# CRIMAC-WP4-Machine-learning/CRIMAC-classifiers-unet

Hardware: AMD Instinct MI355X
Metric: echogram patches/sec (4ch 256x256), training step (fwd+weighted CE+bwd+SGD) (higher is better)
Workload: dtype bf16; 1 GPU; BASELINE configs[1]: U-Net (depth 5, 64 filters) train step, batch 32 x 4x256x256 per GPU; global_batch=32, precision=bf16, start_filts=64, parallelism=dp1, ranks=1, launcher=single process

## Files before the change

### crimac_classifiers_unet_amd/csrc/wgrad.hip

```cpp
#include "common.h"

CRIMAC_DIAG_DECLARE(crimac_diag_clock_wgrad)

namespace {

struct WgradParams {
  const void* f; long f_ld; int CF;
  const void* s; long s_ld; int CS;
  int B, Hf, Wf;
  float* dw;
  int tiles_y, tiles_x;
  long ntiles;
  int tiles_per_block;
  int nsplits;
  long partial_stride;
  int f_es = 2, s_es = 2;
};

__device__ __forceinline__ int swz_tr(int row) { return ((row >> 1) & 1) << 6; }

__device__ __forceinline__ bf16x4 lds_tr16(const unsigned char* p) {
  return __builtin_amdgcn_ds_read_tr16_b64_v4bf16((LDS_PTR(bf16x4))(p));
}

// ... 936 lines not shown
        s_pixel(row, y0, x0, y, x);
        const bool ok = y >= 0 && y < Hs && x >= 0 && x < Ws && (cs0 + u * 8) < p.CS;
        const TA* src = sp + ((b * Hs + y) * (long)Ws + x) * p.s_ld + cs0 + u * 8;
        stage_unit(src, ok, sS, S_BYTES, row * 128 + ((u * 16) ^ swz_tr(row)));
      }
      __syncthreads();
      contract(sF, sS);
    }
  }

  const int col = cs0 + ws * 32 + (lane & 31);
#ifdef CRIMAC_EXP_NOATOMIC
  if (col < 0) {
#else
  if (col < p.CS) {
#endif
    float* dwp = p.dw + (p.partial_stride > 0 ? (long)split * p.partial_stride : 0);
#pragma unroll
    for (int t = 0; t < NTAPS; ++t) {
#pragma unroll
      for (int r = 0; r < 16; ++r) {
        const int row = cf0 + wf * 32 + (r & 3) + 8 * (r >> 2) + 4 * (lane >> 5);
        if (row < p.CF) {
          float* dst = dwp + ((long)t * p.CF + row) * p.CS + col;
          if (p.partial_stride > 0) *dst = acc[t][r];
          else atomicAdd(dst, acc[t][r]);
        }
      }
    }
  }
}

constexpr int kGroupMaxLayers = CRIMAC_WGRAD_GROUP_MAX_LAYERS;
using GroupLayer = crimac_wgrad_group_layer;
struct GroupParams {
  GroupLayer layer[kGroupMaxLayers];
  int B;
  const int* items;
  int cap;
  int count[8];
  unsigned* counter;
  int f_es, s_es;
  int max_items;
};

__device__ __forceinline__ void group_barrier_lds() {
  asm volatile("s_waitcnt lgkmcnt(0)" ::: "memory");
  __builtin_amdgcn_s_barrier();
  asm volatile("" ::: "memory");
}

__device__ __forceinline__ unsigned lds_word(const unsigned* p) {
  return *(volatile LDS_PTR(unsigned))(LDS_PTR(unsigned))(p);
}

template <typename TA>
__global__ __launch_bounds__(512) __attribute__((amdgpu_waves_per_eu(2, 2)))
void wgrad_group_kernel(GroupParams gp) {
  constexpr int MODE = 0, TR = 8, NTAPS = 9;
  constexpr int F_ROWS = TR * 16;
  constexpr int S_ROWS = (TR + 2) * 18;
  constexpr int S_ROWS_PAD = (S_ROWS + 7) / 8 * 8;
  constexpr int F_BYTES = F_ROWS * 128;
  constexpr int S_BYTES = S_ROWS_PAD * 128;
  constexpr int BUF_BYTES = F_BYTES + S_BYTES;
  constexpr int NF = F_ROWS / 8 / 4;
  constexpr int NS = (S_ROWS_PAD / 8 + 3) / 4;
  constexpr unsigned OOB = 0x80000000u;
  extern __shared__ __attribute__((aligned(16))) unsigned char smem[];
  const int tid = threadIdx.x, lane = tid & 63;
  const int team = __builtin_amdgcn_readfirstlane(tid >> 8);
  const int wave = __builtin_amdgcn_readfirstlane((tid >> 6) & 3);
  const int ws = wave & 1, tg = wave >> 1;
  const int g = lane >> 4, li = lane & 15;
  const int q = li >> 2, pp = li & 3;
  const int sub = lane >> 3, c = lane & 7;
  const int xcd = blockIdx.x & 7;
  unsigned* tq = reinterpret_cast<unsigned*>(smem + 4 * BUF_BYTES);
  const int n_items = gp.count[xcd];
  auto fetch_item = [&](int par) {
    const unsigned k = __hip_atomic_fetch_add(gp.counter + xcd, 1u, __ATOMIC_RELAXED, __HIP_MEMORY_SCOPE_AGENT);
    unsigned a = 0, b = 0;
    if (k < (unsigned)n_items) {
      const int* it = gp.items + 2 * ((long)xcd * gp.cap + k);
      a = (unsigned)it[0];
      b = (unsigned)it[1];
    }
    tq[8 + 4 * par] = k;
    tq[9 + 4 * par] = a;
    tq[10 + 4 * par] = b;
  };
  if (tid == 256) fetch_item(0);
  __syncthreads();
  int ipar = 0;

  auto run = [&](auto tgc) {
    constexpr int TG = decltype(tgc)::value;
    using G = WgTaps<MODE, TG>;
    f32x4 acc2[G::N][4][2];
    const int RF = (g >> 1) * 16 + 4 * (g & 1) + q;
    const int RSl = (g >> 1) * G::RS + 4 * (g & 1) + q;
    const unsigned lds0 = (unsigned)(unsigned long)((LDS_PTR(unsigned char))(smem)) + team * 2 * BUF_BYTES;
    const int tt = tid & 255;
    unsigned* tcnt = tq + team;
    for (int taken = 0;; ++taken) {
      const int k = __builtin_amdgcn_readfirstlane((int)lds_word(tq + 8 + 4 * ipar));
      if (k >= n_items) break;
      const int li_ = __builtin_amdgcn_readfirstlane((int)lds_word(tq + 9 + 4 * ipar));
      const int qs = __builtin_amdgcn_readfirstlane((int)lds_word(tq + 10 + 4 * ipar));
      const GroupLayer& p = gp.layer[li_];
      const int qt = qs >> 16, split = qs & 0xFFFF;
      const int cs_tiles = (p.CS + 63) / 64;
      const int cf0 = (qt / cs_tiles) * 64, cs0 = (qt % cs_tiles) * 64;
      const TA* fp = reinterpret_cast<const TA*>(p.f);
      const TA* sp = reinterpret_cast<const TA*>(p.s);
      const int Hs = p.Hf, Ws = p.Wf;
#pragma unroll
      for (int t = 0; t < G::N; ++t)
#pragma unroll
        for (int fh = 0; fh < 4; ++fh)
#pragma unroll
          for (int sh = 0; sh < 2; ++sh)
#pragma unroll
            for (int r = 0; r < 4; ++r) acc2[t][fh][sh][r] = 0.f;
      unsigned f_rel[NF], s_rel[NS];
      auto f_geo = [&](int i, int& ry, int& rx) {
        const int row = 8 * (wave + 4 * i) + sub;
        ry = row >> 4;
        rx = row & 15;
      };
      auto s_geo = [&](int i, int& ry, int& rx) {
        const int row = 8 * (wave + 4 * i) + sub;
        ry = (row * 3641) >> 16;
        rx = row - ry * 18;
      };
#pragma unroll
      for (int i = 0; i < NF; ++i) {
        const int row = 8 * (wave + 4 * i) + sub;
        const int u = c ^ (swz16(row) >> 4);
        int ry, rx;
        f_geo(i, ry, rx);
        f_rel[i] = (cf0 + u * 8) < p.CF ? (unsigned)(((ry * (long)p.Wf + rx) * p.f_ld + cf0 + u * 8) * gp.f_es) : OOB;
      }
#pragma unroll
      for (int i = 0; i < NS; ++i) {
        const int kk = wave + 4 * i;
        const int row = 8 * kk + sub;
        const int u = c ^ (swz16(row) >> 4);
// ... 416 lines not shown
  hipStream_t st = (hipStream_t)stream;
  const bool two = teams_of(prec, mode) == 2;
  if (prec == CRIMAC_PREC_BF16) {
    if (mode == 0 && CS <= 16)
      return two ? launch<bf16_t, 1, 0, true, 2>(p, target_blocks, st) : launch<bf16_t, 1, 0, true>(p, target_blocks, st);
    if (mode == 0) return two ? launch<bf16_t, 1, 0, false, 2>(p, target_blocks, st) : launch<bf16_t, 1, 0>(p, target_blocks, st);
    return launch<bf16_t, 1, 1>(p, target_blocks, st);
  }
  if (prec == CRIMAC_PREC_FP16) {
    if (mode == 0 && CS <= 16)
      return two ? launch<half_t, 1, 0, true, 2>(p, target_blocks, st) : launch<half_t, 1, 0, true>(p, target_blocks, st);
    if (mode == 0) return two ? launch<half_t, 1, 0, false, 2>(p, target_blocks, st) : launch<half_t, 1, 0>(p, target_blocks, st);
    return launch<half_t, 1, 1>(p, target_blocks, st);
  }
  if (prec == CRIMAC_PREC_F32X3)
    return mode == 0 ? launch<float, 2, 0>(p, target_blocks, st) : launch<float, 2, 1>(p, target_blocks, st);
  if (prec == CRIMAC_PREC_H3P) {
    if (pp_ok(prec, mode, CF, CS, f_ld, s_ld, Wf)) return launch_pp(p, target_blocks, st);
    if (up_pp_ok(prec, mode, CF, CS, f_ld, s_ld, Wf, p.partial_stride)) return launch_up_pp(p, target_blocks, st);
    return mode == 0 ? launch<hp_t, 2, 0>(p, target_blocks, st) : launch<hp_t, 2, 1>(p, target_blocks, st);
  }
  return mode == 0 ? launch<float, 3, 0>(p, target_blocks, st) : launch<float, 3, 1>(p, target_blocks, st);
}

}

static int group_check(int prec, const crimac_wgrad_group_layer* L, int n, int B) {
  CRIMAC_REQUIRE(prec == CRIMAC_PREC_BF16 || prec == CRIMAC_PREC_FP16 || prec == CRIMAC_PREC_H3P || prec == CRIMAC_PREC_H3F_BWD,
                 "wgrad_group: 16-bit storage precisions, plane pairs and H3F_BWD only (prec=%d)", prec);
  const bool hp = prec == CRIMAC_PREC_H3P;
  const bool mix = prec == CRIMAC_PREC_H3F_BWD;
  CRIMAC_REQUIRE(L && n >= 1 && n <= CRIMAC_WGRAD_GROUP_MAX_LAYERS && B > 0, "wgrad_group: 1..%d layers", CRIMAC_WGRAD_GROUP_MAX_LAYERS);
  for (int i = 0; i < n; ++i) {
    CRIMAC_REQUIRE(L[i].CF > 0 && L[i].CF % 8 == 0 && L[i].CS >= 64 && L[i].CS % 8 == 0, "wgrad_group: layer %d: CF=%d CS=%d "
                   "(CS >= 64: the first layer keeps its own launch)", i, L[i].CF, L[i].CS);
    CRIMAC_REQUIRE(L[i].f_ld >= L[i].CF && L[i].s_ld >= L[i].CS && L[i].f_ld % 8 == 0 && L[i].s_ld % 8 == 0 && L[i].Hf > 0 && L[i].Wf > 0,
                   "wgrad_group: layer %d: bad strides / sizes", i);
    CRIMAC_REQUIRE((10L * L[i].Wf + 18) * (L[i].f_ld > L[i].s_ld ? L[i].f_ld : L[i].s_ld) * ((hp || mix) ? 4 : 2) < (1L << 31),
                   "wgrad_group: layer %d: a tile's DMA offsets exceed 32 bits", i);
    CRIMAC_REQUIRE(!hp || (L[i].CF % 64 == 0 && L[i].CS % 64 == 0), "wgrad_group: layer %d: plane pairs need whole 64-channel "
                   "tiles (CF=%d CS=%d)", i, L[i].CF, L[i].CS);
  }
  return CRIMAC_OK;
}

extern "C" int crimac_wgrad_group_layer_size(void) { return (int)sizeof(crimac_wgrad_group_layer); }

extern "C" int crimac_wgrad_group_plan(int prec, crimac_wgrad_group_layer* layers, int n_layers, int B, int items_per_layer,
                                       int* items, int cap, int* counts) {
  if (int rc = group_check(prec, layers, n_layers, B)) return rc;
  CRIMAC_REQUIRE(counts, "wgrad_group_plan: counts is NULL");
  static const int env_items = getenv("CRIMAC_WGRAD_GROUP_ITEMS") ? atoi(getenv("CRIMAC_WGRAD_GROUP_ITEMS")) : 0;
  const int target = items_per_layer > 0 ? items_per_layer : (env_items > 0 ? env_items : 128);
  int order[CRIMAC_WGRAD_GROUP_MAX_LAYERS];
  for (int i = 0; i < n_layers; ++i) {
    crimac_wgrad_group_layer& l = layers[i];
    l.tiles_y = cdiv(l.Hf, 8);
    l.tiles_x = cdiv(l.Wf, 16);
    l.ntiles = (long)B * l.tiles_y * l.tiles_x;
    const int ch_tiles = cdiv(l.CF, 64) * cdiv(l.CS, 64);
    long splits = target / ch_tiles;
    const long pix = (long)B * l.Hf * l.Wf;
    long max_splits = pix / 4096 > 1 ? pix / 4096 : 1;
    while (max_splits * ch_tiles < target / 2 && max_splits * 2 <= pix / 1024) max_splits *= 2;
    if (splits > max_splits) splits = max_splits;
    if (splits < 1) splits = 1;
    if (splits > l.ntiles) splits = l.ntiles;
    if (splits >= 8) splits = splits / 8 * 8;
    l.tiles_per_block = cdiv(l.ntiles, splits);
    l.nsplits = cdiv(l.ntiles, l.tiles_per_block);
    CRIMAC_REQUIRE(ch_tiles < 65536 && l.nsplits < 65536, "wgrad_group_plan: layer %d does not fit the item encoding", i);
    order[i] = i;
  }
  for (int a = 1; a < n_layers; ++a)
    for (int b = a; b > 0 && layers[order[b]].tiles_per_block > layers[order[b - 1]].tiles_per_block; --b) {
      const int t = order[b]; order[b] = order[b - 1]; order[b - 1] = t;
    }
  int n[8] = {0, 0, 0, 0, 0, 0, 0, 0};
  long rr = 0;
  for (int oi = 0; oi < n_layers; ++oi) {
    const int li = order[oi];
    const crimac_wgrad_group_layer& l = layers[li];
    const int ch_tiles = cdiv(l.CF, 64) * cdiv(l.CS, 64);
    auto put = [&](int x, int qt, int split) {
      if (items && n[x] < cap) {
        items[2 * ((long)x * cap + n[x])] = li;
        items[2 * ((long)x * cap + n[x]) + 1] = qt * 65536 + split;
      }
      ++n[x];
    };
    if (l.nsplits % 8 == 0) {
      for (int x = 0; x < 8; ++x)
        for (int sp = x; sp < l.nsplits; sp += 8)
          for (int qt = 0; qt < ch_tiles; ++qt) put(x, qt, sp);
    } else {
      for (int sp = 0; sp < l.nsplits; ++sp)
        for (int qt = 0; qt < ch_tiles; ++qt) put((int)(rr++ % 8), qt, sp);
    }
  }
  int need = 0;
  for (int x = 0; x < 8; ++x) { counts[x] = n[x]; if (n[x] > need) need = n[x]; }
  if (items) CRIMAC_REQUIRE(need <= cap, "wgrad_group_plan: %d items per queue, room for %d", need, cap);
  return need;
}

extern "C" int crimac_wgrad_group(int prec, const crimac_wgrad_group_layer* layers, int n_layers, int B, const int* items,
                                  int cap, const int* counts, unsigned int* counters, void* stream) {
  if (int rc = group_check(prec, layers, n_layers, B)) return rc;
  CRIMAC_REQUIRE(items && counts && counters && cap > 0, "wgrad_group: bad queue arguments");
  GroupParams gp;
  for (int i = 0; i < n_layers; ++i) {
    gp.layer[i] = layers[i];
    CRIMAC_REQUIRE(layers[i].f && layers[i].s && layers[i].dw, "wgrad_group: layer %d: NULL tensor", i);
    CRIMAC_REQUIRE(layers[i].tiles_per_block > 0 && layers[i].nsplits > 0 && layers[i].ntiles == (long)B * layers[i].tiles_y * layers[i].tiles_x &&
                       layers[i].tiles_y == cdiv(layers[i].Hf, 8) && layers[i].tiles_x == cdiv(layers[i].Wf, 16),
                   "wgrad_group: layer %d was not planned for this geometry (crimac_wgrad_group_plan)", i);
  }
  gp.B = B; gp.items = items; gp.cap = cap; gp.counter = counters;
  gp.f_es = 2; gp.s_es = prec == CRIMAC_PREC_H3F_BWD ? 4 : 2;
  long total = 0;
  for (int x = 0; x < 8; ++x) {
    CRIMAC_REQUIRE(counts[x] >= 0 && counts[x] <= cap, "wgrad_group: queue %d holds %d items, capacity %d", x, counts[x], cap);
    gp.count[x] = counts[x];
    total += counts[x];
  }
  if (total == 0) return CRIMAC_OK;
  constexpr size_t lds = 4 * (size_t)((8 * 16 + ((8 + 2) * 18 + 7) / 8 * 8) * 128) + 64;
  hipStream_t st = (hipStream_t)stream;
  int ncu = crimac_cu_count();
  ncu = ncu / 8 * 8;
  if (ncu < 8) ncu = 8;
  static const int wg_items = getenv("CRIMAC_WGRAD_GROUP_WGITEMS") ? atoi(getenv("CRIMAC_WGRAD_GROUP_WGITEMS")) : 1;
  gp.max_items = wg_items;
  if (wg_items > 0) {
    int per_xcd = 0;
    for (int x = 0; x < 8; ++x) { const int n = cdiv(counts[x], wg_items); if (n > per_xcd) per_xcd = n; }
    ncu = 8 * per_xcd;
  }
  if (prec == CRIMAC_PREC_H3P) {
    static unsigned long long attr_devs = 0;
    if (crimac_first_use_on_device(&attr_devs))
      (void)hipFuncSetAttribute(reinterpret_cast<const void*>(&wgrad_pp_group_kernel), hipFuncAttributeMaxDynamicSharedMemorySize, 160 * 1024);
    hipLaunchKernelGGL(wgrad_pp_group_kernel, dim3(ncu), dim3(512), 2 * (size_t)PP_BUF + 64, st, gp);
  } else if (prec == CRIMAC_PREC_BF16) {
    static unsigned long long attr_devs = 0;
    if (crimac_first_use_on_device(&attr_devs))
      (void)hipFuncSetAttribute(reinterpret_cast<const void*>(&wgrad_group_kernel<bf16_t>), hipFuncAttributeMaxDynamicSharedMemorySize, 160 * 1024);
    hipLaunchKernelGGL(wgrad_group_kernel<bf16_t>, dim3(ncu), dim3(512), lds, st, gp);
  } else {
    static unsigned long long attr_devs = 0;
    if (crimac_first_use_on_device(&attr_devs))
      (void)hipFuncSetAttribute(reinterpret_cast<const void*>(&wgrad_group_kernel<half_t>), hipFuncAttributeMaxDynamicSharedMemorySize, 160 * 1024);
    hipLaunchKernelGGL(wgrad_group_kernel<half_t>, dim3(ncu), dim3(512), lds, st, gp);
  }
  CRIMAC_LAUNCH_CHECK();
  return CRIMAC_OK;
}

extern "C" int crimac_wgrad(int prec, int mode, const void* f, long f_ld, int CF, const void* s,
                            long s_ld, int CS, int B, int Hf, int Wf, float* dw, int target_blocks,
                            void* stream) {
  return wgrad_run(prec, mode, f, f_ld, CF, s, s_ld, CS, B, Hf, Wf, dw, 0, target_blocks, stream);
}

extern "C" int crimac_wgrad_splits(int prec, int mode, int CF, int CS, int B, int Hf, int Wf, int target_blocks) {
  if (prec < CRIMAC_PREC_BF16 || prec > CRIMAC_PREC_MAX || !(mode == 0 || mode == 1) || CF <= 0 || CS <= 0 || B <= 0 ||
      Hf <= 0 || Wf <= 0)
    return CRIMAC_ERR_INVALID;
  WgradParams p;
  p.CF = CF; p.CS = CS; p.B = B; p.Hf = Hf; p.Wf = Wf;
  plan_splits(p, mode, target_blocks, pp_ok(prec, mode, CF, CS, CF, CS, Wf) ? 2 : teams_of(prec, mode));
  return p.nsplits;
}

extern "C" int crimac_wgrad_partials(int prec, int mode, const void* f, long f_ld, int CF, const void* s,
                                     long s_ld, int CS, int B, int Hf, int Wf, float* partials, long slab_stride,
                                     int target_blocks, void* stream) {
  CRIMAC_REQUIRE(slab_stride > 0, "wgrad_partials: slab_stride must be positive");
  return wgrad_run(prec, mode, f, f_ld, CF, s, s_ld, CS, B, Hf, Wf, partials, slab_stride, target_blocks, stream);
}
```

### crimac_classifiers_unet_amd/engine.py

```python
from __future__ import annotations

import ctypes as C
import os

import torch

from . import hip
from .hip import Act, call, ptr


def _on_device(fn):
    import functools

    @functools.wraps(fn)
    def wrapped(self, *a, **kw):
        if getattr(self, "device", None) is None:
            self.bind()
        dev = self.device
        if dev is None or dev.type != "cuda":
            return fn(self, *a, **kw)
        with torch.cuda.device(dev):
            return fn(self, *a, **kw)
    return wrapped

# ... 377 lines not shown
        if done:
            for gi in range(len(bounds)):
                if gi not in done:
                    self._pack_group(gi)
        else:
            call("crimac_pack_layers", C.byref(arr), len(arr), self._fwd_planes_arg())
            if self.bwd16:
                call("crimac_pack_layers", C.byref(self._ltab16), len(arr), hip.PLANES_FP16)
        self._packed_groups = set()
        self._train_pack_dirty = False

    wgrad_side_streams = int(os.environ.get("CRIMAC_WGRAD_STREAM", "1"))
    unpack_on_side = os.environ.get("CRIMAC_UNPACK_SIDE", "1") != "0"
    early_sgd = os.environ.get("CRIMAC_EARLY_SGD", "1") != "0"
    early_sgd_multi = os.environ.get("CRIMAC_EARLY_SGD_MULTI", "0") != "0"
    exchange_probe = None
    early_pack = os.environ.get("CRIMAC_EARLY_PACK", "1") != "0"
    split_skip_dgrad = os.environ.get("CRIMAC_SPLIT_SKIP", "1") != "0"
    exchange_on_side = os.environ.get("CRIMAC_EXCHANGE_SIDE", "0") != "0"
    _side = None
    _side_events = None
    _eval_side = None

    @staticmethod
    def _gloo_ranks():
        import torch.distributed as dist
        return (dist.is_available() and dist.is_initialized() and dist.get_world_size() > 1
                and dist.get_backend() == "gloo")

    wgrad_group = os.environ.get("CRIMAC_WGRAD_GROUP", "1") != "0"
    wgrad_group_h3p = os.environ.get("CRIMAC_WGRAD_GROUP_H3P", "0") != "0"
    wgrad_group_layers = int(os.environ.get("CRIMAC_WGRAD_GROUP_LAYERS", str(hip.WGRAD_GROUP_MAX_LAYERS)))
    wgrad_group_items = int(os.environ.get("CRIMAC_WGRAD_GROUP_ITEMS", "0"))
    _wg_pending = None

    def _groupable(self, prec, mode, cf, cs):
        if not (self.wgrad_group and mode == 0 and cs >= 64 and not self.use_wgrad_partials and self._wg_pending is not None):
            return False
        if prec == hip.PREC_H3P:
            return self.wgrad_group_h3p and cf % 64 == 0 and cs % 64 == 0
        return prec in hip.PREC_16BIT or prec == hip.PREC_H3F_BWD

    def _group_plan(self, B, shapes):
        key = (self.prec_bwd, B, self.wgrad_group_items, shapes)
        plan = self._wg_plans.get(key)
        if plan is None:
            lib = hip.load_library()
            arr = (hip.WgradGroupLayer * len(shapes))()
            for d, (cf, cs, h, w, f_ld, s_ld) in zip(arr, shapes):
                d.CF, d.CS, d.Hf, d.Wf, d.f_ld, d.s_ld = cf, cs, h, w, f_ld, s_ld
            counts = (C.c_int * 8)()
            cap = lib.crimac_wgrad_group_plan(self.prec_bwd, arr, len(shapes), B, self.wgrad_group_items, None, 0, counts)
            if cap < 0:
                raise hip.HipLibraryError("crimac_wgrad_group_plan failed: " + lib.crimac_last_error().decode(errors="replace"))
            items = torch.zeros(8 * max(cap, 1) * 2, dtype=torch.int32)
            rc = lib.crimac_wgrad_group_plan(self.prec_bwd, arr, len(shapes), B, self.wgrad_group_items,
                                             C.c_void_p(items.data_ptr()), max(cap, 1), counts)
            if rc < 0:
                raise hip.HipLibraryError("crimac_wgrad_group_plan failed: " + lib.crimac_last_error().decode(errors="replace"))
            plan = (arr, items.to(self.device), counts, max(cap, 1))
            self._wg_plans[key] = plan
        return plan

    def _flush_wgrad_group(self):
        pend = self._wg_pending
        if not pend:
            return
        self._wg_pending = []
        B = pend[0]["B"]
        shapes = tuple((q["cf"], q["cs"], q["h"], q["w"], q["f_ld"], q["s_ld"]) for q in pend)
        planned, items_dev, counts, cap = self._group_plan(B, shapes)
        arr = (hip.WgradGroupLayer * len(pend))()
        for d, pl, q in zip(arr, planned, pend):
            C.memmove(C.byref(d), C.byref(pl), C.sizeof(hip.WgradGroupLayer))
            d.f, d.s, d.dw = q["f"].value, q["s"].value, q["dw"].data_ptr()
        if self._wg_launches >= self._wg_counters.numel() // 8:
            raise RuntimeError("more grouped weight-gradient launches in one backward pass than queue counters")
        ctr = ptr(self._wg_counters, 8 * self._wg_launches)
        self._wg_launches += 1
        flops = sum(q["flops"] for q in pend)
        args = (self.prec_bwd, C.byref(arr), len(pend), B, ptr(items_dev), cap, C.byref(counts), ctr)
        self._on_side(lambda: call("crimac_wgrad_group", *args, flops=flops, mfmas=hip.MFMAS_PER_PRODUCT[args[0]]))

    def _on_side(self, fn):
        if self.wgrad_side_streams <= 0 or self._gloo_ranks():
            fn()
            return
        if self._side is None:
            self._side = [torch.cuda.Stream(device=self.device) for _ in range(self.wgrad_side_streams)]
            self._side_events = [torch.cuda.Event() for _ in range(32)]
            self._side_i = 0
        ev = self._side_events[self._side_i % len(self._side_events)]
        side = self._side[self._side_i % len(self._side)]
        self._side_i += 1
        ev.record()
        with torch.cuda.stream(side):
            side.wait_event(ev)
            fn()

    _skip_wgrad = os.environ.get("CRIMAC_EXP_SKIP_WGRAD", "")

    def _wgrad(self, prec, mode, f, f_ld, cf, s_, s_ld, cs, B, h, w, key, flops=None):
        dwt, sp, stride = self._dw(key)
        if self._skip_wgrad == "all" or (self._skip_wgrad == "single" and not self._groupable(prec, mode, cf, cs)):
            return
        if self._groupable(prec, mode, cf, cs):
            self._wg_pending.append(dict(f=f, f_ld=f_ld, cf=cf, s=s_, s_ld=s_ld, cs=cs, B=B, h=h, w=w, dw=dwt,
                                         flops=flops or 0.0))
            if len(self._wg_pending) >= min(self.wgrad_group_layers, hip.WGRAD_GROUP_MAX_LAYERS):
                self._flush_wgrad_group()
            return
        if self.use_wgrad_partials:
            name, args = "crimac_wgrad_partials", (prec, mode, f, f_ld, cf, s_, s_ld, cs, B, h, w, ptr(dwt), stride,
                                                   self.wgrad_target_blocks)
        else:
            name, args = "crimac_wgrad", (prec, mode, f, f_ld, cf, s_, s_ld, cs, B, h, w, ptr(dwt),
                                          self.wgrad_target_blocks)
        self._on_side(lambda: call(name, *args, flops=flops, mfmas=hip.MFMAS_PER_PRODUCT[prec]))

    def _join_wgrad(self):
        if self._side is not None:
            for side in self._side:
                torch.cuda.current_stream().wait_stream(side)

    def _unpack_group(self, gi, on_ready=None, rng=None):
        self._flush_wgrad_group()
        arr, bounds = self._layer_table()
        first, n = bounds[gi]
        side = self._side[0] if (self._side is not None and len(self._side) == 1 and self.unpack_on_side) else None
        if side is not None:
            ev = self._side_events[self._side_i % len(self._side_events)]
            self._side_i += 1
            ev.record()
            with torch.cuda.stream(side):
                side.wait_event(ev)
                if n:
                    call("crimac_unpack_wgrad_layers", C.byref(arr, first * C.sizeof(hip.LayerDesc)), n)
                if on_ready is not None and self.exchange_on_side:
                    on_ready(*rng)
                done = torch.cuda.Event()
                done.record()
                self._unpacked[gi] = done
            if on_ready is not None and not self.exchange_on_side:
                torch.cuda.current_stream().wait_stream(side)
                on_ready(*rng)
            return
        self._join_wgrad()
        if n:
            call("crimac_unpack_wgrad_layers", C.byref(arr, first * C.sizeof(hip.LayerDesc)), n)
        if on_ready is not None:
            on_ready(*rng)
# ... 900 lines not shown
```

### crimac_classifiers_unet_amd/hip.py

```python
from __future__ import annotations

import ctypes as C
import os

import torch

from . import build as _build

PREC_BF16 = 0
PREC_F32X3 = 1
PREC_F32X6 = 2
PREC_FP16 = 3
PREC_F32H3 = 4
PREC_H3P = 5
PREC_H3F_BWD = 6
PREC_NAMES = {"bf16": PREC_BF16, "f32x3": PREC_F32X3, "f32x6": PREC_F32X6, "fp16": PREC_FP16, "f32h3": PREC_F32H3,
              "h3p": PREC_H3P, "h3f": PREC_H3P}
MFMAS_PER_PRODUCT = {PREC_BF16: 1, PREC_FP16: 1, PREC_F32X3: 3, PREC_F32H3: 3, PREC_H3P: 3, PREC_F32X6: 6, PREC_H3F_BWD: 1}
PREC_PLANES = {PREC_BF16: 1, PREC_F32X3: 2, PREC_F32X6: 3, PREC_FP16: 1, PREC_F32H3: 2, PREC_H3P: 2}
PLANES_FP16 = 1 | 16 | 32
PLANES_F32H3 = 2 | 16 | (8 << 8)
PLANES_FWD_FRAG = 65536
PLANES_INTERLEAVED = 64
PLANES_H3P = 2 | 16 | 32 | PLANES_INTERLEAVED | 128 | (8 << 8)
PREC_PLANES_ARG = {PREC_BF16: 1, PREC_F32X3: 2, PREC_F32X6: 3, PREC_FP16: PLANES_FP16, PREC_F32H3: PLANES_F32H3,
                   PREC_H3P: PLANES_H3P}
EPI_RELU, EPI_OUT_PLANES, EPI_CIN4 = 1, 2, 4
EPI_WFRAG = 16
EPI_WROWS = 32
LAYER_FWD_FRAG, LAYER_DG_FRAG = 16, 32
PREC_BACKWARD = {PREC_F32H3: PREC_F32X3}
PREC_16BIT = (PREC_BF16, PREC_FP16)

ABI_VERSION = 6

_vp, _i, _l, _f = C.c_void_p, C.c_int, C.c_long, C.c_float

SIGNATURES = {
    "crimac_igemm_conv": [_i, _vp, _l, _i, _i, _i, _i, _i, _i, _i, _i, _i, _i, _i, _vp, _vp, _vp, _i,
                          _vp, _l, _i, _i, _i, _vp],
    "crimac_conv3x3": [_i, _vp, _l, _i, _i, _i, _i, _i, _vp, _vp, _vp, _vp, _l, _i, _i, _vp, _vp, _i,
                       _vp, _l, _vp, _l, _vp],
    "crimac_conv3x3_pool": [_i, _vp, _l, _i, _i, _i, _i, _i, _vp, _vp, _vp, _vp, _l, _i, _vp, _l, _vp],
    "crimac_conv3x3_cols": [_i, _vp, _l, _i, _i, _i, _i, _i, _vp, _vp, _vp, _vp, _l, _i, _i, _vp, _vp, _i,
                            _vp, _l, _vp, _l, _i, _i, _vp],
    "crimac_upconv2x2_dgrad_bnb": [_vp, _l, _i, _i, _i, _i, _i, _vp, _vp, _l, _vp, _l, _vp, _l, _vp, _vp, _i, _vp],
    "crimac_upconv2x2_dgrad_bnb_prec": [_i, _vp, _l, _i, _i, _i, _i, _i, _vp, _vp, _l, _vp, _l, _vp, _l, _vp, _vp, _i,
                                        _vp],
    "crimac_sum_replicas": [_vp, _i, _l, _i, _vp, _vp, _vp, _vp, _vp],
    "crimac_wgrad": [_i, _i, _vp, _l, _i, _vp, _l, _i, _i, _i, _i, _vp, _i, _vp],
    "crimac_wgrad_partials": [_i, _i, _vp, _l, _i, _vp, _l, _i, _i, _i, _i, _vp, _l, _i, _vp],
    "crimac_wgrad_group": [_i, _vp, _i, _i, _vp, _i, _vp, _vp, _vp],
    "crimac_pack_conv3x3": [_vp, _i, _i, _i, _vp, _i, _vp, _vp, _vp, _vp, _vp],
    "crimac_pack_upconv2x2": [_vp, _i, _i, _i, _vp, _vp, _vp, _vp, _vp],
    "crimac_unpack_wgrad_conv3x3": [_vp, _i, _i, _i, _vp, _vp],
    "crimac_unpack_wgrad_upconv2x2": [_vp, _i, _i, _vp, _vp],
    "crimac_pack_layers": [_vp, _i, _i, _vp],
    "crimac_unpack_wgrad_layers": [_vp, _i, _vp],
    "crimac_nchw_to_nhwc": [_i, _vp, _vp, _i, _i, _i, _i, _l, _vp],
    "crimac_colstats": [_i, _vp, _l, _l, _i, _vp, _vp, _vp],
    "crimac_colsum_f32": [_i, _vp, _l, _l, _i, _vp, _vp],
    "crimac_bn_finalize": [_vp, _vp, _i, _l, _i, _vp, _vp, _f, _f, _vp, _vp, _vp, _vp, _vp, _vp, _vp, _vp],
    "crimac_bn_act_pool": [_i, _vp, _l, _vp, _vp, _i, _vp, _l, _vp, _l, _i, _i, _i, _i, _vp],
    "crimac_bn_train_act_pool": [_i, _vp, _l, _vp, _vp, _i, _l, _vp, _vp, _f, _f, _vp, _vp, _vp, _vp, _l, _i, _vp, _l,
                                 _vp, _l, _i, _i, _i, _i, _vp],
    "crimac_unpool_add": [_i, _vp, _l, _vp, _l, _vp, _l, _vp, _l, _i, _i, _i, _i, _vp, _l, _vp, _l, _vp, _vp, _i,
                          _vp],
# ... 14 lines not shown
    "crimac_sgd_momentum_guarded": [_vp, _vp, _vp, _l, _f, _f, _f, _i, _vp, _vp],
    "crimac_meta_planes": [_vp, _i, _i, _i, _i, C.c_double, _vp, _i, _vp, _i, _vp, _i, _vp, _vp],
    "crimac_meta_mlp_fwd": [_vp, _i, _i, _i, _i, _vp, _vp, _vp, _vp, _vp, _vp, _vp, _vp],
    "crimac_meta_inject_fwd": [_vp, _vp, _vp, _i, _i, _i, _i, _i, _vp],
    "crimac_meta_bwd": [_vp, _vp, _i, _i, _i, _i, _i, _vp, _vp, _vp, _vp, _vp, _vp, _vp, _vp, _vp, _vp, _vp, _vp, _vp,
                        _vp, _vp],
    "crimac_gather_patches": [_i, _vp, _i, _i, _i, _vp, _i, _i, _i, _vp, _l, _vp],
    "crimac_gather_patches_memm": [_i, _vp, _i, _i, _i, _vp, _i, _i, _i, _vp, _l, _vp, _vp],
    "crimac_scatter_patches_ex": [_vp, _i, _vp, _i, _i, _i, _i, _i, _i, _i, _vp, _vp, _i, _i, _vp, _i, _i, _vp, _i, _i,
                                  _i, _i, _vp, _i, _vp],
    "crimac_augment_db_nhwc": [_i, _vp, _vp, _i, _vp, _vp, _vp, _i, _f, _f, _i, _i, _i, _i, _l, C.c_ulonglong,
                               _i, _i, _i, _vp],
    "crimac_augment_flip_planes": [_vp, _vp, _i, _i, _i, _i, C.c_ulonglong, _i, _vp],
    "crimac_refine_labels": [_vp, _i, _vp, _vp, _i, _f, _f, _i, _vp, _i, _i, _i, _i, _vp],
    "crimac_pr_histogram": [_vp, _i, _vp, _i, _i, _i, _i, _vp, _vp, _vp],
    "crimac_mfma_calibrate": [_i, _i, _vp, _vp],
    "crimac_labels_test_transform": [_vp, _i, _vp, _i, _f, _f, _vp, _vp, _i, _i, _vp, _i, _i, _i, _i, _i, _i, _vp, _i, _i,
                                     _i, _i],
    "crimac_labels_extend_mask": [_vp, _vp, _i, _vp, _vp, _i, _i, _i, _i, _i],
    "crimac_scatter_patches": [_vp, _i, _vp, _i, _i, _i, _i, _i, _i, _i, _vp, _vp, _i, _i, _vp, _i, _i,
                               _i, _vp, _vp],
}



class LayerDesc(C.Structure):
    _fields_ = [("w", _vp), ("grad", _vp), ("dw", _vp), ("fwd_hi", _vp), ("fwd_lo", _vp), ("dg_hi", _vp),
                ("dg_lo", _vp), ("kind", _i), ("Co", _i), ("Ci", _i), ("Ci_pad", _i), ("dw_splits", _i),
                ("dw_stride", _l)]


class WgradGroupLayer(C.Structure):
    _fields_ = [("f", _vp), ("f_ld", _l), ("CF", _i), ("s", _vp), ("s_ld", _l), ("CS", _i), ("Hf", _i), ("Wf", _i),
                ("dw", _vp), ("tiles_y", _i), ("tiles_x", _i), ("ntiles", _l), ("tiles_per_block", _i), ("nsplits", _i)]


WGRAD_GROUP_MAX_LAYERS = 16
MASK_PER_PATCH = -2147483648


_lib = None


class HipLibraryError(RuntimeError):
    pass


def library_path() -> str:
    return os.environ.get("CRIMAC_LIB") or _build.LIB_PATH


def load_library():
    global _lib
    if _lib is not None:
        return _lib
    path = library_path()
    if not os.path.exists(path):
        raise HipLibraryError(
            f"{path} is missing: build it with `python -m crimac_classifiers_unet_amd.build` "
            "(hipcc, gfx950). There is no CPU fallback for the U-Net hot path.")
    lib = C.CDLL(path)
    lib.crimac_version.restype = C.c_int
    lib.crimac_version.argtypes = []
    lib.crimac_last_error.restype = C.c_char_p
    lib.crimac_last_error.argtypes = []
    ver = lib.crimac_version()
    if ver != ABI_VERSION:
        raise HipLibraryError(f"{path} has ABI version {ver}, this binding needs {ABI_VERSION}: rebuild it "
                              "(`python -m crimac_classifiers_unet_amd.build --force`)")
    if not hasattr(lib, "crimac_layer_desc_size"):
# ... 73 lines not shown
```

### include/crimac_unet_hip.h

```cpp
#ifndef CRIMAC_UNET_HIP_H_
#define CRIMAC_UNET_HIP_H_

#ifdef __cplusplus
extern "C" {
#endif

#define CRIMAC_OK 0
#define CRIMAC_ERR_INVALID (-22)
#define CRIMAC_ERR_LAUNCH (-5)

#define CRIMAC_PREC_BF16 0
#define CRIMAC_PREC_F32X3 1
#define CRIMAC_PREC_F32X6 2
#define CRIMAC_PREC_FP16 3
#define CRIMAC_PREC_F32H3 4
#define CRIMAC_PREC_H3P 5
#define CRIMAC_PREC_MAX 5
#define CRIMAC_PREC_H3F_BWD 6
#define CRIMAC_F32H3_WSHIFT 8
#define CRIMAC_PLANES_FWD_FP16 16
#define CRIMAC_PLANES_DG_FP16 32
#define CRIMAC_PLANES_FP16 (1 | CRIMAC_PLANES_FWD_FP16 | CRIMAC_PLANES_DG_FP16)
#define CRIMAC_PLANES_F32H3 (2 | CRIMAC_PLANES_FWD_FP16 | (CRIMAC_F32H3_WSHIFT << 8))
#define CRIMAC_PLANES_INTERLEAVED 64
#define CRIMAC_PLANES_FWD_FRAG 65536
#define CRIMAC_PLANES_DG_SCALED 128
#define CRIMAC_PLANES_H3P (2 | CRIMAC_PLANES_FWD_FP16 | CRIMAC_PLANES_DG_FP16 | CRIMAC_PLANES_INTERLEAVED | \
                           CRIMAC_PLANES_DG_SCALED | (CRIMAC_F32H3_WSHIFT << 8))

#define CRIMAC_EPI_RELU 1
#define CRIMAC_EPI_OUT_PLANES 2
#define CRIMAC_EPI_CIN4 4
#define CRIMAC_EPI_STAT_RAW 8
#define CRIMAC_EPI_WFRAG 16
#define CRIMAC_EPI_WROWS 32

#define CRIMAC_ABI_VERSION 6
int crimac_version(void);
int crimac_layer_desc_size(void);
const char* crimac_last_error(void);


int crimac_igemm_conv(int prec, const void* in, long in_ld, int B, int Hi, int Wi, int Ho, int Wo,
                      int Cin, int N, int ntaps, int tw, int pad, int stride, const void* w_hi,
                      const void* w_lo, const float* bias, int bias_mod, void* out, long out_ld,
                      int relu, int out_mode, int cout_up, void* stream);

int crimac_upconv2x2_dgrad_bnb(const void* dy, long dy_ld, int B, int H, int W, int Cout, int Cin,
                               const void* w_dg_hi, void* dx, long dx_ld, const void* bnb_y, long bnb_y_ld,
                               const float* bnb_vec, long bnb_stride, double* stat_sum, double* stat_sumsq,
                               int stat_replicas, void* stream);
int crimac_upconv2x2_dgrad_bnb_prec(int prec, const void* dy, long dy_ld, int B, int H, int W, int Cout, int Cin,
                                    const void* w_dg_hi, void* dx, long dx_ld, const void* bnb_y, long bnb_y_ld,
                                    const float* bnb_vec, long bnb_stride, double* stat_sum, double* stat_sumsq,
                                    int stat_replicas, void* stream);


int crimac_conv3x3(int prec, const void* in, long in_ld, int B, int H, int W, int Cin, int N,
                   const void* w_hi, const void* w_lo, const float* bias, void* out, long out_ld,
                   int relu, int stat_mode, double* stat_sum, double* stat_sumsq, int stat_replicas,
                   const void* bnb_y, long bnb_y_ld, const float* bnb_vec, long bnb_stride, void* stream);

int crimac_conv3x3_cols(int prec, const void* in, long in_ld, int B, int H, int W, int Cin, int N,
                   const void* w_hi, const void* w_lo, const float* bias, void* out, long out_ld,
                   int relu, int stat_mode, double* stat_sum, double* stat_sumsq, int stat_replicas,
                   const void* bnb_y, long bnb_y_ld, const float* bnb_vec, long bnb_stride, int n_first, int n_count, void* stream);

int crimac_conv3x3_pool(int prec, const void* in, long in_ld, int B, int H, int W, int Cin, int N,
                        const void* w_hi, const void* w_lo, const float* bias, void* out, long out_ld, int relu,
                        void* pool_out, long pool_ld, void* stream);

int crimac_wgrad(int prec, int mode, const void* f, long f_ld, int CF, const void* s, long s_ld,
                 int CS, int B, int Hf, int Wf, float* dw, int target_blocks, void* stream);

#define CRIMAC_WGRAD_GROUP_MAX_LAYERS 16
typedef struct crimac_wgrad_group_layer {
  const void* f; long f_ld; int CF;
  const void* s; long s_ld; int CS;
  int Hf, Wf;
  float* dw;
  int tiles_y, tiles_x;
  long ntiles;
  int tiles_per_block, nsplits;
} crimac_wgrad_group_layer;
int crimac_wgrad_group_layer_size(void);
int crimac_wgrad_group_plan(int prec, crimac_wgrad_group_layer* layers, int n_layers, int B, int items_per_layer,
                            int* items, int cap, int* counts);
int crimac_wgrad_group(int prec, const crimac_wgrad_group_layer* layers, int n_layers, int B, const int* items, int cap,
                       const int* counts, unsigned int* counters, void* stream);
int crimac_wgrad_splits(int prec, int mode, int CF, int CS, int B, int Hf, int Wf, int target_blocks);
int crimac_wgrad_partials(int prec, int mode, const void* f, long f_ld, int CF, const void* s, long s_ld, int CS,
                          int B, int Hf, int Wf, float* partials, long slab_stride, int target_blocks, void* stream);



int crimac_pack_conv3x3(const float* w, int Co, int Ci, int Ci_pad, const float* scale, int planes,
                        void* fwd_hi, void* fwd_lo, void* dg_hi, void* dg_lo, void* stream);
int crimac_pack_upconv2x2(const float* w, int Ci, int Co, int planes, void* fwd_hi, void* fwd_lo,
                          void* dg_hi, void* dg_lo, void* stream);
int crimac_unpack_wgrad_conv3x3(const float* dw, int Co, int Ci, int Ci_pad, float* grad, void* stream);
int crimac_unpack_wgrad_upconv2x2(const float* dw, int Ci, int Co, float* grad, void* stream);

typedef struct crimac_layer_desc {
  const float* w;
  float* grad;
  const float* dw;
  void* fwd_hi;
  void* fwd_lo;
  void* dg_hi;
  void* dg_lo;
  int kind;
  int Co, Ci, Ci_pad;
  int dw_splits;
  long dw_stride;
} crimac_layer_desc;
#define CRIMAC_LAYER_FWD_FRAG 16
// ... 140 lines not shown
```

Measured before the change: 2949 patches/s.

## Fold upconv2x2 weight-gradient work into the grouped wgrad persistent kernel

Adds a second item kind (2x2 up-convolution, mode 1) to the grouped weight-gradient kernel, with its own tile geometry (4-row tiles, 128-channel F blocks, double-buffered LDS DMA) so upconv wgrads share the persistent work queue with the conv3x3 layers. The intent is to remove separate upconv wgrad launches and fill idle CUs during the grouped launch. The planner now orders layers by an estimated per-kind cost. The trade-off is extra kernel variants and register/code pressure in the templated kernel. Groups that contain only upconv layers still fall back to single launches.

```diff
diff --git a/crimac_classifiers_unet_amd/csrc/wgrad.hip b/crimac_classifiers_unet_amd/csrc/wgrad.hip
--- a/crimac_classifiers_unet_amd/csrc/wgrad.hip
+++ b/crimac_classifiers_unet_amd/csrc/wgrad.hip
@@ -992,6 +992,9 @@
 }
 
 constexpr int kGroupMaxLayers = CRIMAC_WGRAD_GROUP_MAX_LAYERS;
+constexpr int UG_F_IMG = 64 * 128;
+constexpr int UG_S_IMG = 256 * 128;
+constexpr int UG_BUF = 2 * UG_F_IMG + UG_S_IMG;
 using GroupLayer = crimac_wgrad_group_layer;
 struct GroupParams {
   GroupLayer layer[kGroupMaxLayers];
@@ -1014,7 +1017,7 @@
   return *(volatile LDS_PTR(unsigned))(LDS_PTR(unsigned))(p);
 }
 
-template <typename TA>
+template <typename TA, bool UP>
 __global__ __launch_bounds__(512) __attribute__((amdgpu_waves_per_eu(2, 2)))
 void wgrad_group_kernel(GroupParams gp) {
   constexpr int MODE = 0, TR = 8, NTAPS = 9;
@@ -1037,6 +1040,7 @@
   const int sub = lane >> 3, c = lane & 7;
   const int xcd = blockIdx.x & 7;
   unsigned* tq = reinterpret_cast<unsigned*>(smem + 4 * BUF_BYTES);
+  static_assert(2 * UG_BUF <= 4 * BUF_BYTES, "kind-1 tile buffers below the queue words");
   const int n_items = gp.count[xcd];
   auto fetch_item = [&](int par) {
     const unsigned k = __hip_atomic_fetch_add(gp.counter + xcd, 1u, __ATOMIC_RELAXED, __HIP_MEMORY_SCOPE_AGENT);
@@ -1069,11 +1073,115 @@
       const int li_ = __builtin_amdgcn_readfirstlane((int)lds_word(tq + 9 + 4 * ipar));
       const int qs = __builtin_amdgcn_readfirstlane((int)lds_word(tq + 10 + 4 * ipar));
       const GroupLayer& p = gp.layer[li_];
+      const int kind = __builtin_amdgcn_readfirstlane(p.kind);
       const int qt = qs >> 16, split = qs & 0xFFFF;
       const int cs_tiles = (p.CS + 63) / 64;
-      const int cf0 = (qt / cs_tiles) * 64, cs0 = (qt % cs_tiles) * 64;
       const TA* fp = reinterpret_cast<const TA*>(p.f);
       const TA* sp = reinterpret_cast<const TA*>(p.s);
+      if (UP && kind == 1) {
+        using U = WgTaps<1, TG>;
+#pragma unroll
+        for (int t = 0; t < U::N; ++t)
+#pragma unroll
+          for (int fh = 0; fh < 4; ++fh)
+#pragma unroll
+            for (int sh = 0; sh < 2; ++sh)
+#pragma unroll
+              for (int r = 0; r < 4; ++r) acc2[t][fh][sh][r] = 0.f;
+        const long t_begin = (long)split * p.tiles_per_block;
+        const long t_end = t_begin + p.tiles_per_block < p.ntiles ? t_begin + p.tiles_per_block : p.ntiles;
+        const bool last = gp.max_items > 0 && taken + 1 >= gp.max_items;
+        const int w8 = team * 4 + wave;
+        const int cf0 = (qt / cs_tiles) * 128, cs0 = (qt % cs_tiles) * 64;
+        const int Hs = 2 * p.Hf, Ws = 2 * p.Wf;
+        unsigned f_rel[2], s_rel[4];
+#pragma unroll
+        for (int i = 0; i < 2; ++i) {
+          const int kk = w8 + 8 * i, row = 8 * (kk & 7) + sub;
+          const int u = c ^ (swz16(row) >> 4);
+          const int ch = cf0 + 64 * (kk >> 3) + u * 8;
+          f_rel[i] = ch < p.CF ? (unsigned)((((row >> 4) * (long)p.Wf + (row & 15)) * p.f_ld + ch) * 2) : OOB;
+        }
+#pragma unroll
+        for (int i = 0; i < 4; ++i) {
+          const int row = 8 * (w8 + 8 * i) + sub;
+          const int u = c ^ (swz16(row) >> 4);
+          const int ch = cs0 + u * 8;
+          s_rel[i] = ch < p.CS ? (unsigned)((((row >> 5) * (long)Ws + 2 * (row & 15) + ((row >> 4) & 1)) * p.s_ld + ch) * 2)
+                               : OOB;
+        }
+        auto issue_up = [&](long tile, int buf) {
+          const int txi = (int)(tile % p.tiles_x);
+          const long ttl = tile / p.tiles_x;
+          const int y0 = (int)(ttl % p.tiles_y) * 4, x0 = txi * 16;
+          const long b = ttl / p.tiles_y;
+          unsigned char* base = smem + buf * UG_BUF;
+          const __amdgpu_buffer_rsrc_t rf = __builtin_amdgcn_make_buffer_rsrc(
+              const_cast<char*>(reinterpret_cast<const char*>(fp) + ((b * p.Hf + y0) * (long)p.Wf + x0) * p.f_ld * 2), 0,
+              0x7FFFFFFF, 0x00020000);
+#pragma unroll
+          for (int i = 0; i < 2; ++i) {
+            const int kk = w8 + 8 * i, row = 8 * (kk & 7) + sub;
+            const bool ok = (y0 + (row >> 4)) < p.Hf && (x0 + (row & 15)) < p.Wf;
+            __builtin_amdgcn_raw_ptr_buffer_load_lds(rf, (__attribute__((address_space(3))) void*)(base + kk * 1024), 16,
+                                                     (int)(ok ? f_rel[i] : OOB), 0, 0, 0);
+          }
+          const __amdgpu_buffer_rsrc_t rs = __builtin_amdgcn_make_buffer_rsrc(
+              const_cast<char*>(reinterpret_cast<const char*>(sp) + ((b * Hs + 2 * y0) * (long)Ws + 2 * x0) * p.s_ld * 2), 0,
+              0x7FFFFFFF, 0x00020000);
+#pragma unroll
+          for (int i = 0; i < 4; ++i) {
+            const int kk = w8 + 8 * i, row = 8 * kk + sub;
+            const bool ok = (y0 + (row >> 6)) < p.Hf && (x0 + (row & 15)) < p.Wf;
+            __builtin_amdgcn_raw_ptr_buffer_load_lds(rs, (__attribute__((address_space(3))) void*)(base + 2 * UG_F_IMG + kk * 1024),
+                                                     16, (int)(ok ? s_rel[i] : OOB), 0, 0, 0);
+          }
+        };
+        const int RSu = (g >> 1) * U::RS + 4 * (g & 1) + q;
+        const unsigned ldsw = (unsigned)(unsigned long)((LDS_PTR(unsigned char))(smem));
+        issue_up(t_begin, 0);
+        if (tid == 256) {
+          if (last) tq[8 + 4 * (ipar ^ 1)] = 0x7FFFFFFFu;
+          else fetch_item(ipar ^ 1);
+        }
+        for (long tile = t_begin; tile < t_end; ++tile) {
+          const int cur = (int)((tile - t_begin) & 1);
+          asm volatile("s_waitcnt vmcnt(0)" ::: "memory");
+          group_barrier_lds();
+          if (tile + 1 < t_end) issue_up(tile + 1, cur ^ 1);
+          const unsigned aF = ldsw + cur * UG_BUF + team * UG_F_IMG, aS = ldsw + cur * UG_BUF + 2 * UG_F_IMG;
+          const unsigned fv0 = aF + RF * 128 + 8 * pp + swz16(RF);
+          unsigned sv[4];
+#pragma unroll
+          for (int kk = 0; kk < 4; ++kk) sv[kk] = aS + RSu * 128 + 8 * pp + ((ws * 64) ^ swz16(kk + RSu));
+          WgFrags f;
+          wg_rd_a<0, 0>(fv0, f);
+          wg_rd_a<0, 1>(fv0, f);
+          wg_rd_a<0, 2>(fv0, f);
+          wg_rd_a<0, 3>(fv0, f);
+          wg_rd_b<1, TG, 0, false>(sv, f);
+          wg_step<typename PlaneOf<TA>::type, 1, TG, 0, false>(fv0, sv, f, acc2);
+        }
+        group_barrier_lds();
+        ipar ^= 1;
+#pragma unroll
+        for (int sh = 0; sh < 2; ++sh) {
+          const int col = cs0 + ws * 32 + sh * 16 + (lane & 15);
+          if (col < p.CS) {
+#pragma unroll
+            for (int t = 0; t < U::N; ++t)
+#pragma unroll
+              for (int fh = 0; fh < 4; ++fh)
+#pragma unroll
+                for (int r = 0; r < 4; ++r) {
+                  const int row = cf0 + 64 * team + fh * 16 + (lane >> 4) * 4 + r;
+                  if (row < p.CF) atomicAdd(p.dw + ((long)(U::T0 + t) * p.CF + row) * p.CS + col, acc2[t][fh][sh][r]);
+                }
+          }
+        }
+        continue;
+      }
+      const int cf0 = (qt / cs_tiles) * 64, cs0 = (qt % cs_tiles) * 64;
       const int Hs = p.Hf, Ws = p.Wf;
 #pragma unroll
       for (int t = 0; t < G::N; ++t)
@@ -1556,16 +1664,33 @@
   const bool mix = prec == CRIMAC_PREC_H3F_BWD;
   CRIMAC_REQUIRE(L && n >= 1 && n <= CRIMAC_WGRAD_GROUP_MAX_LAYERS && B > 0, "wgrad_group: 1..%d layers", CRIMAC_WGRAD_GROUP_MAX_LAYERS);
   for (int i = 0; i < n; ++i) {
+    const int kind = L[i].kind;
+    CRIMAC_REQUIRE(kind == CRIMAC_WGRAD_KIND_CONV3X3 || kind == CRIMAC_WGRAD_KIND_UP2X2, "wgrad_group: layer %d: bad kind %d",
+                   i, kind);
+    CRIMAC_REQUIRE(kind == CRIMAC_WGRAD_KIND_CONV3X3 || prec == CRIMAC_PREC_BF16 || prec == CRIMAC_PREC_FP16,
+                   "wgrad_group: layer %d: kind %d needs 16-bit storage (bf16 / fp16)", i, kind);
     CRIMAC_REQUIRE(L[i].CF > 0 && L[i].CF % 8 == 0 && L[i].CS >= 64 && L[i].CS % 8 == 0, "wgrad_group: layer %d: CF=%d CS=%d "
                    "(CS >= 64: the first layer keeps its own launch)", i, L[i].CF, L[i].CS);
     CRIMAC_REQUIRE(L[i].f_ld >= L[i].CF && L[i].s_ld >= L[i].CS && L[i].f_ld % 8 == 0 && L[i].s_ld % 8 == 0 && L[i].Hf > 0 && L[i].Wf > 0,
                    "wgrad_group: layer %d: bad strides / sizes", i);
-    CRIMAC_REQUIRE((10L * L[i].Wf + 18) * (L[i].f_ld > L[i].s_ld ? L[i].f_ld : L[i].s_ld) * ((hp || mix) ? 4 : 2) < (1L << 31),
-                   "wgrad_group: layer %d: a tile's DMA offsets exceed 32 bits", i);
+    if (kind == CRIMAC_WGRAD_KIND_UP2X2)
+      CRIMAC_REQUIRE((4L * L[i].Wf + 16) * L[i].f_ld * 2 < (1L << 31) && (16L * L[i].Wf + 32) * L[i].s_ld * 2 < (1L << 31),
+                     "wgrad_group: layer %d: a tile's DMA offsets exceed 32 bits", i);
+    else
+      CRIMAC_REQUIRE((10L * L[i].Wf + 18) * (L[i].f_ld > L[i].s_ld ? L[i].f_ld : L[i].s_ld) * ((hp || mix) ? 4 : 2) < (1L << 31),
+                     "wgrad_group: layer %d: a tile's DMA offsets exceed 32 bits", i);
     CRIMAC_REQUIRE(!hp || (L[i].CF % 64 == 0 && L[i].CS % 64 == 0), "wgrad_group: layer %d: plane pairs need whole 64-channel "
                    "tiles (CF=%d CS=%d)", i, L[i].CF, L[i].CS);
   }
   return CRIMAC_OK;
+}
+
+static int group_tile_rows(int kind) { return kind == CRIMAC_WGRAD_KIND_UP2X2 ? 4 : 8; }
+static int group_ch_tiles(const crimac_wgrad_group_layer& l) {
+  return cdiv(l.CF, l.kind == CRIMAC_WGRAD_KIND_UP2X2 ? 128 : 64) * cdiv(l.CS, 64);
+}
+static long group_cost(const crimac_wgrad_group_layer& l) {
+  return (long)l.tiles_per_block * (l.kind == CRIMAC_WGRAD_KIND_UP2X2 ? 7 : 16);
 }
 
 extern "C" int crimac_wgrad_group_layer_size(void) { return (int)sizeof(crimac_wgrad_group_layer); }
@@ -1579,10 +1704,10 @@
   int order[CRIMAC_WGRAD_GROUP_MAX_LAYERS];
   for (int i = 0; i < n_layers; ++i) {
     crimac_wgrad_group_layer& l = layers[i];
-    l.tiles_y = cdiv(l.Hf, 8);
+    l.tiles_y = cdiv(l.Hf, group_tile_rows(l.kind));
     l.tiles_x = cdiv(l.Wf, 16);
     l.ntiles = (long)B * l.tiles_y * l.tiles_x;
-    const int ch_tiles = cdiv(l.CF, 64) * cdiv(l.CS, 64);
+    const int ch_tiles = group_ch_tiles(l);
     long splits = target / ch_tiles;
     const long pix = (long)B * l.Hf * l.Wf;
     long max_splits = pix / 4096 > 1 ? pix / 4096 : 1;
@@ -1597,7 +1722,7 @@
     order[i] = i;
   }
   for (int a = 1; a < n_layers; ++a)
-    for (int b = a; b > 0 && layers[order[b]].tiles_per_block > layers[order[b - 1]].tiles_per_block; --b) {
+    for (int b = a; b > 0 && group_cost(layers[order[b]]) > group_cost(layers[order[b - 1]]); --b) {
       const int t = order[b]; order[b] = order[b - 1]; order[b - 1] = t;
     }
   int n[8] = {0, 0, 0, 0, 0, 0, 0, 0};
@@ -1605,7 +1730,7 @@
   for (int oi = 0; oi < n_layers; ++oi) {
     const int li = order[oi];
     const crimac_wgrad_group_layer& l = layers[li];
-    const int ch_tiles = cdiv(l.CF, 64) * cdiv(l.CS, 64);
+    const int ch_tiles = group_ch_tiles(l);
     auto put = [&](int x, int qt, int split) {
       if (items && n[x] < cap) {
         items[2 * ((long)x * cap + n[x])] = li;
@@ -1637,7 +1762,8 @@
     gp.layer[i] = layers[i];
     CRIMAC_REQUIRE(layers[i].f && layers[i].s && layers[i].dw, "wgrad_group: layer %d: NULL tensor", i);
     CRIMAC_REQUIRE(layers[i].tiles_per_block > 0 && layers[i].nsplits > 0 && layers[i].ntiles == (long)B * layers[i].tiles_y * layers[i].tiles_x &&
-                       layers[i].tiles_y == cdiv(layers[i].Hf, 8) && layers[i].tiles_x == cdiv(layers[i].Wf, 16),
+                       layers[i].tiles_y == cdiv(layers[i].Hf, group_tile_rows(layers[i].kind)) &&
+                       layers[i].tiles_x == cdiv(layers[i].Wf, 16),
                    "wgrad_group: layer %d was not planned for this geometry (crimac_wgrad_group_plan)", i);
   }
   gp.B = B; gp.items = items; gp.cap = cap; gp.counter = counters;
@@ -1666,16 +1792,24 @@
     if (crimac_first_use_on_device(&attr_devs))
       (void)hipFuncSetAttribute(reinterpret_cast<const void*>(&wgrad_pp_group_kernel), hipFuncAttributeMaxDynamicSharedMemorySize, 160 * 1024);
     hipLaunchKernelGGL(wgrad_pp_group_kernel, dim3(ncu), dim3(512), 2 * (size_t)PP_BUF + 64, st, gp);
-  } else if (prec == CRIMAC_PREC_BF16) {
-    static unsigned long long attr_devs = 0;
-    if (crimac_first_use_on_device(&attr_devs))
-      (void)hipFuncSetAttribute(reinterpret_cast<const void*>(&wgrad_group_kernel<bf16_t>), hipFuncAttributeMaxDynamicSharedMemorySize, 160 * 1024);
-    hipLaunchKernelGGL(wgrad_group_kernel<bf16_t>, dim3(ncu), dim3(512), lds, st, gp);
   } else {
-    static unsigned long long attr_devs = 0;
-    if (crimac_first_use_on_device(&attr_devs))
-      (void)hipFuncSetAttribute(reinterpret_cast<const void*>(&wgrad_group_kernel<half_t>), hipFuncAttributeMaxDynamicSharedMemorySize, 160 * 1024);
-    hipLaunchKernelGGL(wgrad_group_kernel<half_t>, dim3(ncu), dim3(512), lds, st, gp);
+    bool up = false;
+    for (int i = 0; i < n_layers; ++i) up = up || layers[i].kind == CRIMAC_WGRAD_KIND_UP2X2;
+    const void* fn = prec == CRIMAC_PREC_BF16
+                         ? (up ? reinterpret_cast<const void*>(&wgrad_group_kernel<bf16_t, true>)
+                               : reinterpret_cast<const void*>(&wgrad_group_kernel<bf16_t, false>))
+                         : (up ? reinterpret_cast<const void*>(&wgrad_group_kernel<half_t, true>)
+                               : reinterpret_cast<const void*>(&wgrad_group_kernel<half_t, false>));
+    static unsigned long long attr_devs[2][2] = {{0, 0}, {0, 0}};
+    if (crimac_first_use_on_device(&attr_devs[prec == CRIMAC_PREC_BF16][up]))
+      (void)hipFuncSetAttribute(fn, hipFuncAttributeMaxDynamicSharedMemorySize, 160 * 1024);
+    if (prec == CRIMAC_PREC_BF16) {
+      if (up) hipLaunchKernelGGL((wgrad_group_kernel<bf16_t, true>), dim3(ncu), dim3(512), lds, st, gp);
+      else hipLaunchKernelGGL((wgrad_group_kernel<bf16_t, false>), dim3(ncu), dim3(512), lds, st, gp);
+    } else {
+      if (up) hipLaunchKernelGGL((wgrad_group_kernel<half_t, true>), dim3(ncu), dim3(512), lds, st, gp);
+      else hipLaunchKernelGGL((wgrad_group_kernel<half_t, false>), dim3(ncu), dim3(512), lds, st, gp);
+    }
   }
   CRIMAC_LAUNCH_CHECK();
   return CRIMAC_OK;
diff --git a/crimac_classifiers_unet_amd/engine.py b/crimac_classifiers_unet_amd/engine.py
--- a/crimac_classifiers_unet_amd/engine.py
+++ b/crimac_classifiers_unet_amd/engine.py
@@ -433,11 +433,14 @@
     wgrad_group_h3p = os.environ.get("CRIMAC_WGRAD_GROUP_H3P", "0") != "0"
     wgrad_group_layers = int(os.environ.get("CRIMAC_WGRAD_GROUP_LAYERS", str(hip.WGRAD_GROUP_MAX_LAYERS)))
     wgrad_group_items = int(os.environ.get("CRIMAC_WGRAD_GROUP_ITEMS", "0"))
+    wgrad_group_fold = os.environ.get("CRIMAC_WGRAD_GROUP_FOLD", "1") != "0"
     _wg_pending = None
 
     def _groupable(self, prec, mode, cf, cs):
-        if not (self.wgrad_group and mode == 0 and cs >= 64 and not self.use_wgrad_partials and self._wg_pending is not None):
+        if not (self.wgrad_group and cs >= 64 and not self.use_wgrad_partials and self._wg_pending is not None):
             return False
+        if mode == 1:
+            return self.wgrad_group_fold and prec in hip.PREC_16BIT
         if prec == hip.PREC_H3P:
             return self.wgrad_group_h3p and cf % 64 == 0 and cs % 64 == 0
         return prec in hip.PREC_16BIT or prec == hip.PREC_H3F_BWD
@@ -448,8 +451,8 @@
         if plan is None:
             lib = hip.load_library()
             arr = (hip.WgradGroupLayer * len(shapes))()
-            for d, (cf, cs, h, w, f_ld, s_ld) in zip(arr, shapes):
-                d.CF, d.CS, d.Hf, d.Wf, d.f_ld, d.s_ld = cf, cs, h, w, f_ld, s_ld
+            for d, (cf, cs, h, w, f_ld, s_ld, kind) in zip(arr, shapes):
+                d.CF, d.CS, d.Hf, d.Wf, d.f_ld, d.s_ld, d.kind = cf, cs, h, w, f_ld, s_ld, kind
             counts = (C.c_int * 8)()
             cap = lib.crimac_wgrad_group_plan(self.prec_bwd, arr, len(shapes), B, self.wgrad_group_items, None, 0, counts)
             if cap < 0:
@@ -468,8 +471,12 @@
         if not pend:
             return
         self._wg_pending = []
+        if all(q["kind"] != hip.WGRAD_KIND_CONV3X3 for q in pend):
+            for q in pend:
+                q["single"]()
+            return
         B = pend[0]["B"]
-        shapes = tuple((q["cf"], q["cs"], q["h"], q["w"], q["f_ld"], q["s_ld"]) for q in pend)
+        shapes = tuple((q["cf"], q["cs"], q["h"], q["w"], q["f_ld"], q["s_ld"], q["kind"]) for q in pend)
         planned, items_dev, counts, cap = self._group_plan(B, shapes)
         arr = (hip.WgradGroupLayer * len(pend))()
         for d, pl, q in zip(arr, planned, pend):
@@ -505,19 +512,26 @@
         dwt, sp, stride = self._dw(key)
         if self._skip_wgrad == "all" or (self._skip_wgrad == "single" and not self._groupable(prec, mode, cf, cs)):
             return
-        if self._groupable(prec, mode, cf, cs):
-            self._wg_pending.append(dict(f=f, f_ld=f_ld, cf=cf, s=s_, s_ld=s_ld, cs=cs, B=B, h=h, w=w, dw=dwt,
-                                         flops=flops or 0.0))
-            if len(self._wg_pending) >= min(self.wgrad_group_layers, hip.WGRAD_GROUP_MAX_LAYERS):
-                self._flush_wgrad_group()
-            return
         if self.use_wgrad_partials:
             name, args = "crimac_wgrad_partials", (prec, mode, f, f_ld, cf, s_, s_ld, cs, B, h, w, ptr(dwt), stride,
                                                    self.wgrad_target_blocks)
         else:
             name, args = "crimac_wgrad", (prec, mode, f, f_ld, cf, s_, s_ld, cs, B, h, w, ptr(dwt),
                                           self.wgrad_target_blocks)
-        self._on_side(lambda: call(name, *args, flops=flops, mfmas=hip.MFMAS_PER_PRODUCT[prec]))
+
+        def single():
+            self._on_side(lambda: call(name, *args, flops=flops, mfmas=hip.MFMAS_PER_PRODUCT[prec]))
+        if self._groupable(prec, mode, cf, cs):
+            kind = hip.WGRAD_KIND_UP2X2 if mode == 1 else hip.WGRAD_KIND_CONV3X3
+            if len(self._wg_pending) >= hip.WGRAD_GROUP_MAX_LAYERS:
+                self._flush_wgrad_group()
+            self._wg_pending.append(dict(f=f, f_ld=f_ld, cf=cf, s=s_, s_ld=s_ld, cs=cs, B=B, h=h, w=w, dw=dwt,
+                                         flops=flops or 0.0, kind=kind, single=single))
+            n3 = sum(q["kind"] == hip.WGRAD_KIND_CONV3X3 for q in self._wg_pending)
+            if n3 >= min(self.wgrad_group_layers, hip.WGRAD_GROUP_MAX_LAYERS):
+                self._flush_wgrad_group()
+            return
+        single()
 
     def _join_wgrad(self):
         if self._side is not None:
diff --git a/crimac_classifiers_unet_amd/hip.py b/crimac_classifiers_unet_amd/hip.py
--- a/crimac_classifiers_unet_amd/hip.py
+++ b/crimac_classifiers_unet_amd/hip.py
@@ -32,7 +32,7 @@
 PREC_BACKWARD = {PREC_F32H3: PREC_F32X3}
 PREC_16BIT = (PREC_BF16, PREC_FP16)
 
-ABI_VERSION = 6
+ABI_VERSION = 7
 
 _vp, _i, _l, _f = C.c_void_p, C.c_int, C.c_long, C.c_float
 
@@ -113,10 +113,12 @@
 
 class WgradGroupLayer(C.Structure):
     _fields_ = [("f", _vp), ("f_ld", _l), ("CF", _i), ("s", _vp), ("s_ld", _l), ("CS", _i), ("Hf", _i), ("Wf", _i),
-                ("dw", _vp), ("tiles_y", _i), ("tiles_x", _i), ("ntiles", _l), ("tiles_per_block", _i), ("nsplits", _i)]
+                ("dw", _vp), ("tiles_y", _i), ("tiles_x", _i), ("ntiles", _l), ("tiles_per_block", _i), ("nsplits", _i),
+                ("kind", _i)]
 
 
 WGRAD_GROUP_MAX_LAYERS = 16
+WGRAD_KIND_CONV3X3, WGRAD_KIND_UP2X2 = 0, 1
 MASK_PER_PATCH = -2147483648
 
 
diff --git a/include/crimac_unet_hip.h b/include/crimac_unet_hip.h
--- a/include/crimac_unet_hip.h
+++ b/include/crimac_unet_hip.h
@@ -35,7 +35,7 @@
 #define CRIMAC_EPI_WFRAG 16
 #define CRIMAC_EPI_WROWS 32
 
-#define CRIMAC_ABI_VERSION 6
+#define CRIMAC_ABI_VERSION 7
 int crimac_version(void);
 int crimac_layer_desc_size(void);
 const char* crimac_last_error(void);
@@ -74,6 +74,8 @@
                  int CS, int B, int Hf, int Wf, float* dw, int target_blocks, void* stream);
 
 #define CRIMAC_WGRAD_GROUP_MAX_LAYERS 16
+#define CRIMAC_WGRAD_KIND_CONV3X3 0
+#define CRIMAC_WGRAD_KIND_UP2X2 1
 typedef struct crimac_wgrad_group_layer {
   const void* f; long f_ld; int CF;
   const void* s; long s_ld; int CS;
@@ -82,6 +84,7 @@
   int tiles_y, tiles_x;
   long ntiles;
   int tiles_per_block, nsplits;
+  int kind;
 } crimac_wgrad_group_layer;
 int crimac_wgrad_group_layer_size(void);
 int crimac_wgrad_group_plan(int prec, crimac_wgrad_group_layer* layers, int n_layers, int B, int items_per_layer,
```

New measurement: 2990 patches/s, median of 6. 1.4% higher.
